# nmerty/nerf-fl

Hardware: AMD Instinct MI355X
Metric: ray-samples/sec (64+64) (higher is better)
Workload: dtype f16x3 fwd + f16 bwd; 1 GPU; configs[1]: lego-like rays, base NeRF coarse+fine, white_back; 4096 rays/GPU, N_samples=64 + N_importance=64, perturb=1 noise_std=1; train step: render_rays fwd + NerfWLoss + HIP backward + grad all-reduce + Adam + re-pack; rays_per_gpu=4096, mode=train, precision=f16x3, forward_arithmetic=fp16 MFMA, operands split hi+lo, 3 products, fp32 accumulate (f16x3), mlp_evals_per_ray=192, hip_graph=False, full=False

## Files before the change

### nerf_fl_amd/csrc/nfl_math.h

```cpp
#pragma once
#include <hip/hip_runtime.h>

#include "../../include/nerf_fl_amd.h"
#include "nfl_macros.h"

typedef float f4v __attribute__((ext_vector_type(4)));

template <class Cam>
NFL_DEV void nfl_cam_ray(const Cam& c, long long p, f4v& r0, f4v& r1) {
    const float i = (float)(p % c.width), j = (float)(p / c.width);
    const float dx = (i - c.cx) / c.fx, dy = -(j - c.cy) / c.fy, dz = -1.f;
    float d[3];
#pragma unroll
    for (int r = 0; r < 3; ++r) d[r] = dx * c.c2w[4 * r] + dy * c.c2w[4 * r + 1] + dz * c.c2w[4 * r + 2];
    const float n = sqrtf(d[0] * d[0] + d[1] * d[1] + d[2] * d[2]);
    r0 = f4v{c.c2w[3], c.c2w[7], c.c2w[11], d[0] / n};
    r1 = f4v{d[1] / n, d[2] / n, c.near, c.far};
}

NFL_DEV float nfl_softplus(float x) { return x > 20.f ? x : log1pf(expf(x)); }
NFL_DEV float nfl_sigmoid(float x) { return 1.f / (1.f + expf(-x)); }

NFL_DEV float nfl_sin_rev(float r) {
    r = r - rintf(r);
    float a = fabsf(r);
    a = a > 0.25f ? 0.5f - a : a;
    a = copysignf(a, r);
    const float a2 = a * a;
    float p = 3.953670604e+01f;
    p = __builtin_fmaf(p, a2, -7.654978229e+01f);
    p = __builtin_fmaf(p, a2, 8.160100407e+01f);
    p = __builtin_fmaf(p, a2, -4.134165503e+01f);
    p = __builtin_fmaf(p, a2, 6.283185160e+00f);
    return a * p;
}

NFL_DEV void nfl_turns(float x, float& th, float& tl) {
    const float C_HI = 0.15915493667125702f;
    const float C_LO = 6.4206382432985265e-09f;
    th = x * C_HI;
    const float e = __builtin_fmaf(x, C_HI, -th);
    tl = __builtin_fmaf(x, C_LO, e);
}

template <int N>
NFL_DEV float nfl_pe_feature(int f, const float (&raw)[3], const float (&th)[3], const float (&tl)[3], const float* pw) {
    if (f < 3) return raw[f];
    if (f >= 6 * N + 3) return 0.f;
    const int g = f - 3, k = g / 6, rem = g % 6, t = rem / 3, c = rem % 3;
    const float sc = (float)(1 << k);
    float r = __builtin_amdgcn_fractf(th[c] * sc) + tl[c] * sc;
    if (t) r += 0.25f;
    return pw[k] * nfl_sin_rev(r);
}

NFL_DEV float nfl_relu(float x) {
    int b = __builtin_bit_cast(int, x);
    b = b > 0 ? b : 0;
    return __builtin_bit_cast(float, b);
}
template <class E>
NFL_DEV unsigned nfl_pack2(float a, float b) {
    typedef E e2v __attribute__((ext_vector_type(2)));
    e2v r;
    r[0] = (E)a;
    r[1] = (E)b;
    return __builtin_bit_cast(unsigned, r);
}
template <class E>
NFL_DEV unsigned nfl_split_pair(float x0, float x1, float& l0, float& l1) {
    const unsigned hi = nfl_pack2<E>(x0, x1);
    if constexpr (__is_same(E, _Float16)) {
        asm("v_fma_mix_f32 %0, %1, -1.0, %2 op_sel_hi:[1,0,0]" : "=v"(l0) : "v"(hi), "v"(x0));
        asm("v_fma_mix_f32 %0, %1, -1.0, %2 op_sel:[1,0,0] op_sel_hi:[1,0,0]" : "=v"(l1) : "v"(hi), "v"(x1));
    } else {
        l0 = x0 - __builtin_bit_cast(float, hi << 16);
        asm volatile("" : "+v"(l0));
        l1 = x1 - __builtin_bit_cast(float, hi & 0xffff0000u);
    }
    return hi;
}

template <int NP>
NFL_DEV void nfl_split8(const float (&v)[8], h8 (&dst)[NP]) {
    using E = _Float16;
#pragma unroll
    for (int j = 0; j < 8; j += 2) {
        if constexpr (NP == 2) {
            float l0, l1;
            reinterpret_cast<unsigned(&)[4]>(dst[0])[j / 2] = nfl_split_pair<E>(v[j], v[j + 1], l0, l1);
            reinterpret_cast<unsigned(&)[4]>(dst[NP - 1])[j / 2] = nfl_pack2<E>(l0, l1);
        } else {
            reinterpret_cast<unsigned(&)[4]>(dst[0])[j / 2] = nfl_pack2<E>(v[j], v[j + 1]);
        }
    }
}
```

### nerf_fl_amd/csrc/nfl_mlp.h

```cpp
#pragma once
#include "nfl_dev.h"
#include "nfl_diag.h"
#include "nfl_math.h"
#include "nfl_plan.h"
#include "nfl_prods.h"

__device__ __forceinline__ f16v nfl_mfma(h8 a, h8 b, f16v c) { return __builtin_amdgcn_mfma_f32_32x32x16_f16(a, b, c, 0, 0, 0); }

#define NFL_STREAM_STORE(v, p) __builtin_nontemporal_store(v, p)

template <int LO = 0>
NFL_DEV void nfl_stash8(const float (&v)[8], char* dst) {
    h8 t, tl;
#pragma unroll
    for (int j = 0; j < 8; j += 2) {
        if constexpr (LO != 0) {
            float l0, l1;
            reinterpret_cast<unsigned(&)[4]>(t)[j / 2] = nfl_split_pair<_Float16>(v[j], v[j + 1], l0, l1);
            reinterpret_cast<unsigned(&)[4]>(tl)[j / 2] = nfl_pack2<_Float16>(l0, l1);
        } else {
            reinterpret_cast<unsigned(&)[4]>(t)[j / 2] = nfl_pack2<_Float16>(v[j], v[j + 1]);
        }
    }
    NFL_STREAM_STORE(t, reinterpret_cast<h8*>(dst));
    if constexpr (LO != 0) NFL_STREAM_STORE(tl, reinterpret_cast<h8*>(dst + LO));
}

template <int N, int NP, int LO = 0>
NFL_DEV void nfl_pe_kstep(int ks, int h, const float (&raw)[3], const float (&th)[3], const float (&tl)[3],
                          const float* pw, h8 (&dst)[NP], char* stash = nullptr) {
    float v[8];
#pragma unroll
    for (int j = 0; j < 8; ++j) {
        const int f0 = 16 * ks + j, f1 = f0 + 8;
        if (f0 < 3 || f0 >= 6 * N + 3 || f1 >= 6 * N + 3) {
            const float v0 = nfl_pe_feature<N>(f0, raw, th, tl, pw);
            const float v1 = nfl_pe_feature<N>(f1, raw, th, tl, pw);
            v[j] = h ? v1 : v0;
        } else {
            const int g0 = f0 - 3, g1 = f1 - 3;
            const int k0 = g0 / 6, k1 = g1 / 6, t0 = (g0 % 6) / 3, t1 = (g1 % 6) / 3, c0 = g0 % 3, c1 = g1 % 3;
            const float sc = h ? (float)(1 << k1) : (float)(1 << k0);
            const float thc = h ? th[c1] : th[c0];
            const float tlc = h ? tl[c1] : tl[c0];
            const float ph = h ? 0.25f * t1 : 0.25f * t0;
            const float r = __builtin_amdgcn_fractf(thc * sc) + tlc * sc + ph;
            v[j] = (h ? pw[k1] : pw[k0]) * nfl_sin_rev(r);
        }
    }
    nfl_split8<NP>(v, dst);
    if (stash) {
        NFL_STREAM_STORE(dst[0], reinterpret_cast<h8*>(stash));
        if constexpr (LO != 0 && NP == 2) NFL_STREAM_STORE(dst[NP - 1], reinterpret_cast<h8*>(stash + LO));
    }
}

template <int SLOT_BYTES, int MAXP_>
struct NflRing {
    static constexpr int MAXP = MAXP_;
    const char* gsrc;
    const int* chunk_off;
    char* lds;
    int n_chunks;
    int c_issue;
    int s_issue;
    int s_read;
    int wave, lane;
    const char* i_src;
    char* i_dst;
    int i_nbytes;

#ifdef NFL_STAMPS
    unsigned long long t_wait = 0, t_bar = 0;
#endif
    int n_off0, n_off1;
    unsigned ovf = 0;

    NFL_DEV void begin_issue() {
        i_nbytes = n_off1 - n_off0;
        i_src = gsrc + n_off0;
        i_dst = lds + s_issue * SLOT_BYTES;
        c_issue = c_issue + 1 == n_chunks ? 0 : c_issue + 1;
        s_issue = s_issue == 2 ? 0 : s_issue + 1;
        n_off0 = __builtin_amdgcn_readfirstlane(chunk_off[c_issue]);
        n_off1 = __builtin_amdgcn_readfirstlane(chunk_off[c_issue + 1]);
    }
    template <int P>
    NFL_DEV void piece() {
        if constexpr (P < MAXP) {
            unsigned byte = (unsigned)(wave + 4 * P) * 1024u;
            const unsigned last = (unsigned)i_nbytes - 1024u;
            byte = byte < last ? byte : last;
            const unsigned vo = byte + (threadIdx.x & 63) * 16u;
            __builtin_amdgcn_global_load_lds(
                (const __attribute__((address_space(1))) void*)(i_src + vo),
                (__attribute__((address_space(3))) void*)(i_dst + byte), 16, 0, 0);
        }
    }
    template <int P0, int P1>
    NFL_DEV void pieces() {
        nfl_static_for<P0, P1>([&](auto P) __attribute__((always_inline)) { piece<decltype(P)::value>(); });
    }
    NFL_DEV void prime() {
        n_off0 = __builtin_amdgcn_readfirstlane(chunk_off[c_issue]);
        n_off1 = __builtin_amdgcn_readfirstlane(chunk_off[c_issue + 1]);
        begin_issue();
        pieces<0, MAXP>();
        begin_issue();
        pieces<0, MAXP>();
    }
    template <int EXTRA = 0>
    NFL_DEV const char* consume() {
#if defined(NFL_STAMPS) && NFL_STAMPS >= 2
        const unsigned long long c0 = __builtin_amdgcn_s_memtime();
        asm volatile("s_waitcnt vmcnt(%0) lgkmcnt(0)" ::"n"(MAXP + EXTRA) : "memory");
        const unsigned long long c1 = __builtin_amdgcn_s_memtime();
        __builtin_amdgcn_s_barrier();
        t_wait += c1 - c0;
        t_bar += __builtin_amdgcn_s_memtime() - c1;
#else
        asm volatile("s_waitcnt vmcnt(%0) lgkmcnt(0)" ::"n"(MAXP + EXTRA) : "memory");
        __builtin_amdgcn_s_barrier();
#endif
        asm volatile("" ::: "memory");
        begin_issue();
        const char* base = lds + s_read * SLOT_BYTES + (threadIdx.x & 63) * 16;
        s_read = s_read == 2 ? 0 : s_read + 1;
        return base;
    }
};

template <int NP, int NCB>
NFL_DEV void nfl_bias_init(f16v (&acc)[NCB], const float* bias_rt, int h) {
#pragma unroll
    for (int q = 0; q < 4; ++q) {
        const f4v b = *reinterpret_cast<const f4v*>(bias_rt + 8 * q + 4 * h);
#pragma unroll
        for (int cb = 0; cb < NCB; ++cb) {
            acc[cb][4 * q + 0] = b[0];
            acc[cb][4 * q + 1] = b[1];
            acc[cb][4 * q + 2] = b[2];
            acc[cb][4 * q + 3] = b[3];
        }
    }
}

typedef unsigned nfl_u4 __attribute__((ext_vector_type(4)));
template <int OFF>
NFL_DEV nfl_u4 nfl_lds_read128(unsigned addr) {
    static_assert(OFF >= 0 && OFF < 65536, "ds_read offset field is 16 bits");
    nfl_u4 r;
    asm volatile("ds_read_b128 %0, %1 offset:%2" : "=v"(r) : "v"(addr), "n"(OFF));
    return r;
}
template <int N, int NREAD, int NWP>
NFL_DEV void nfl_lds_wait(nfl_u4 (&w)[NWP]) {
    if constexpr (NREAD == 2) asm volatile("s_waitcnt lgkmcnt(%2)" : "+v"(w[0]), "+v"(w[1]) : "n"(N));
    else asm volatile("s_waitcnt lgkmcnt(%1)" : "+v"(w[0]) : "n"(N));
}

#ifndef NFL_DEPTH_X3
#define NFL_DEPTH_X3 2
#endif
template <int PRODS, int NP, int NCB, int NK, int P0, class V8, class GetB, class Epi, class Ring,
          int DEPTH = ((NP == 1 && (PRODS & 4) == 0) ? 4 : NFL_DEPTH_X3)>
NFL_DEV void nfl_tile_p(f16v (&acc)[NCB], const char* wl, const int frag0, GetB&& getb, Epi&& epi, Ring& ring) {
    constexpr int NWP = (NP == 2 || (PRODS & 4) != 0) ? 2 : 1;
    constexpr int KSB = 1024 * NWP;
    constexpr int NW = DEPTH + 1;
    constexpr bool W_LO = NWP == 2 && (PRODS & 1) != 0, X_LO = NP == 2 && (PRODS & 2) != 0;
    constexpr int NREAD = W_LO ? 2 : 1;
    (void)frag0;
    nfl_u4 w[NW][NWP];
    const unsigned wa = (unsigned)(size_t)(__attribute__((address_space(3))) const char*)wl;
    auto load = [&](auto K) __attribute__((always_inline)) {
        constexpr int k = decltype(K)::value;
        w[k % NW][0] = nfl_lds_read128<(P0 + k) * KSB>(wa);
        if constexpr (W_LO) w[k % NW][NWP - 1] = nfl_lds_read128<(P0 + k) * KSB + 1024>(wa);
    };
    nfl_static_for<0, (DEPTH < NK ? DEPTH : NK)>([&](auto K) __attribute__((always_inline)) { load(K); });
    epi.early();
    __builtin_amdgcn_sched_barrier(0);
    nfl_static_for<0, NK>([&](auto K) __attribute__((always_inline)) {
        constexpr int k = decltype(K)::value;
        constexpr int younger = (NK - 1 - k) < (DEPTH - 1) ? (NK - 1 - k) : (DEPTH - 1);
        nfl_lds_wait<younger * NREAD, NREAD>(w[k % NW]);
#pragma unroll
        for (int cb = 0; cb < NCB; ++cb) {
            if constexpr (W_LO) {
                acc[cb] = nfl_mfma(__builtin_bit_cast(V8, w[k % NW][NWP - 1]), getb(K, cb, 0), acc[cb]);
                if (cb == 0) {
                    if constexpr (k + DEPTH < NK) load(std::integral_constant<int, k + DEPTH>{});
                }
                __builtin_amdgcn_sched_barrier(0);
            }
            if constexpr (X_LO) {
                acc[cb] = nfl_mfma(__builtin_bit_cast(V8, w[k % NW][0]), getb(K, cb, NP - 1), acc[cb]);
                if (cb == 0) {
                    if constexpr (!W_LO && k + DEPTH < NK) load(std::integral_constant<int, k + DEPTH>{});
                    ring.template piece<P0 + k>();
                }
                __builtin_amdgcn_sched_barrier(0);
            }
            acc[cb] = nfl_mfma(__builtin_bit_cast(V8, w[k % NW][0]), getb(K, cb, 0), acc[cb]);
            if (cb == 0) {
                if constexpr (!W_LO && !X_LO && k + DEPTH < NK) load(std::integral_constant<int, k + DEPTH>{});
                if constexpr (!X_LO) ring.template piece<P0 + k>();
            }
            if (cb == NCB - 1) epi.template step<k, NK>();
            __builtin_amdgcn_sched_barrier(0);
        }
    });
}
template <int NP, int NCB, int NK, int P0, class V8, class GetB, class Epi, class Ring>
NFL_DEV void nfl_tile(f16v (&acc)[NCB], const char* wl, const int frag0, GetB&& getb, Epi&& epi, Ring& ring) {
    nfl_tile_p<3, NP, NCB, NK, P0, V8>(acc, wl, frag0, getb, epi, ring);
}

struct NflNoEpi {
    template <int K, int NK> NFL_DEV void step() {}
    NFL_DEV void early() {}
};
#ifndef NFL_EPI_EARLY
#define NFL_EPI_EARLY 2
#endif

template <int NP, int NCB, bool RELU, bool STASH, int NOUT, int MSLOT, int LO = 0, bool ZST = false>
struct NflActEpi {
    const f16v (&acc)[NCB];
    h8 (&out)[NOUT][NCB][NP];
    const int ks;
    char* const (&stash)[NCB];
    const int slot;
    char* const (&mstash)[NCB];
    const int mword;
    unsigned (&mq)[NCB][4];
    unsigned& ovf;
    float* const* zc;
    const int zpad;
    h8 tmp[NCB];
    h8 tmpl[LO != 0 ? NCB : 1];
    unsigned m32[NCB];

    template <int OP>
    NFL_DEV void pair() {
        constexpr int s = OP / 4, j = 2 * (OP % 4);
#pragma unroll
        for (int cb = 0; cb < NCB; ++cb) {
            float x0 = acc[cb][8 * s + j], x1 = acc[cb][8 * s + j + 1];
            if constexpr (ZST) {
                const int f = 16 * (ks + s) + 8 * (j >> 2) + 4 * (int)((threadIdx.x & 63) >> 5) + (j & 3);
                zc[cb][(size_t)f * zpad] = x0;
                zc[cb][(size_t)(f + 1) * zpad] = x1;
            }
            if (RELU) {
                x0 = nfl_relu(x0);
                x1 = nfl_relu(x1);
            }
            unsigned hi;
            if constexpr (NP == 2) {
                float l0, l1;
                hi = nfl_split_pair<_Float16>(x0, x1, l0, l1);
                const unsigned lo = nfl_pack2<_Float16>(l0, l1);
                reinterpret_cast<unsigned(&)[4]>(out[ks + s][cb][NP - 1])[j / 2] = lo;
                if constexpr (STASH && LO != 0) {
                    reinterpret_cast<unsigned(&)[4]>(tmpl[cb])[j / 2] = lo;
                    if (OP % 4 == 3) NFL_STREAM_STORE(tmpl[cb], reinterpret_cast<h8*>(stash[cb] + LO + (slot + s) * 1024));
                }
            } else {
                hi = nfl_pack2<_Float16>(x0, x1);
            }
            reinterpret_cast<unsigned(&)[4]>(out[ks + s][cb][0])[j / 2] = hi;
            {
                const unsigned mag = RELU ? hi : (hi & 0x7fff7fffu);
                asm("v_pk_max_u16 %0, %0, %1" : "+v"(ovf) : "v"(mag));
            }
            if (STASH) {
                reinterpret_cast<unsigned(&)[4]>(tmp[cb])[j / 2] = hi;
                if (OP % 4 == 3) NFL_STREAM_STORE(tmp[cb], reinterpret_cast<h8*>(stash[cb] + (slot + s) * 1024));
                if (RELU) {
                    unsigned on;
                    asm("v_pk_min_u16 %0, %1, %2" : "=v"(on) : "v"(hi), "s"(0x00010001u));
                    m32[cb] = OP == 0 ? on : ((on << (2 * OP)) | m32[cb]);
                    if (OP == 7) {
                        mq[cb][MSLOT] = m32[cb];
                        if (MSLOT == 3) {
                            typedef unsigned nfl_mq4 __attribute__((ext_vector_type(4)));
                            const nfl_mq4 v = {mq[cb][0], mq[cb][1], mq[cb][2], mq[cb][3]};
                            NFL_STREAM_STORE(v, reinterpret_cast<nfl_mq4*>(mstash[cb] + (mword >> 2) * 1024));
                        }
                    }
                }
            }
        }
    }
    template <int K, int NK>
    NFL_DEV void step() {
        constexpr int R = 8 - NFL_EPI_EARLY;
        nfl_static_for<NFL_EPI_EARLY + (R * K) / NK, NFL_EPI_EARLY + (R * (K + 1)) / NK>([&](auto O) __attribute__((always_inline)) {
            pair<decltype(O)::value>();
        });
    }
    NFL_DEV void early() {
        nfl_static_for<0, NFL_EPI_EARLY>([&](auto O) __attribute__((always_inline)) { pair<decltype(O)::value>(); });
    }
    NFL_DEV void all() {
        nfl_static_for<0, 8>([&](auto O) __attribute__((always_inline)) { pair<decltype(O)::value>(); });
    }
};

template <int NP, int NCB, int NKA, int NKB, bool RELU, int NRT, int TPC, bool STASH, int LO = 0, int PRODS = 3, bool ZST = false, int NINA, int NINB, int NOUT, class Ring>
NFL_DEV void nfl_dense(Ring& ring, const float* bias_lds, int& rt, int h,
                       const h8 (&inA)[NINA][NCB][NP], int ksA0,
                       const h8 (&inB)[NINB][NCB][NP], int ksB0,
                       h8 (&out)[NOUT][NCB][NP], int out_ks0, char* const (&stash)[NCB], int slot0,
                       char* const (&mstash)[NCB], int mw0, float* const* zc = nullptr, int zpad = 0) {
    constexpr int NK = NKA + NKB;
    constexpr int NST = 2 * NCB * (LO != 0 ? 2 : 1);
    unsigned mq[NCB][4];
    f16v acc[2][NCB];
    const char* wl = nullptr;
    auto getb = [&](auto K, int cb, int part) __attribute__((always_inline)) -> const h8& {
        constexpr int k = decltype(K)::value;
        if constexpr (k < NKA) return inA[ksA0 + k][cb][part];
        else return inB[ksB0 + k - NKA][cb][part];
    };
    nfl_static_for<0, NRT>([&](auto I) __attribute__((always_inline)) {
        constexpr int i = decltype(I)::value;
        if (i % TPC == 0) wl = ring.template consume<(STASH && TPC == 1 && i >= 2) ? NST : 0>();
        constexpr int frag0 = (i % TPC) * NK;
        nfl_bias_init<NP, NCB>(acc[i & 1], bias_lds + (rt + i) * 32, h);
        if constexpr (i > 0) {
            NflActEpi<NP, NCB, RELU, STASH, NOUT, (i - 1) & 3, LO, ZST> epi{acc[(i - 1) & 1], out, out_ks0 + 2 * (i - 1), stash, slot0 + 2 * (i - 1), mstash, mw0 + i - 1, mq, ring.ovf, zc, zpad};
            nfl_tile_p<PRODS, NP, NCB, NK, frag0, h8>(acc[i & 1], wl, frag0, getb, epi, ring);
        } else {
            NflNoEpi epi;
            nfl_tile_p<PRODS, NP, NCB, NK, frag0, h8>(acc[i & 1], wl, frag0, getb, epi, ring);
        }
        if (i % TPC == TPC - 1 || i == NRT - 1) ring.template pieces<((i % TPC) + 1) * NK, Ring::MAXP>();
    });
    NflActEpi<NP, NCB, RELU, STASH, NOUT, (NRT - 1) & 3, LO, ZST> last{acc[(NRT - 1) & 1], out, out_ks0 + 2 * (NRT - 1), stash, slot0 + 2 * (NRT - 1), mstash, mw0 + NRT - 1, mq, ring.ovf, zc, zpad};
    last.all();
    rt += NRT;
}

template <int NP, int NCB, int NK, int PRODS = 3, int NIN, class Ring>
NFL_DEV void nfl_head(Ring& ring, const float* bias_lds, int& rt, int h,
                      const h8 (&in)[NIN][NCB][NP], int ks0, f16v (&acc)[NCB]) {
    const char* wl = ring.consume();
    nfl_bias_init<NP, NCB>(acc, bias_lds + rt * 32, h);
    auto getb = [&](auto K, int cb, int part) __attribute__((always_inline)) -> const h8& {
        return in[ks0 + decltype(K)::value][cb][part];
    };
    NflNoEpi epi;
    nfl_tile_p<PRODS, NP, NCB, NK, 0, h8>(acc, wl, 0, getb, epi, ring);
    ring.template pieces<NK, Ring::MAXP>();
    rt += 1;
}
```

### nerf_fl_amd/csrc/nfl_render_impl.h

```cpp
#pragma once
#include "nfl_launch.h"
#include "nfl_mlp.h"

#define NFL_NST 20
#define NFL_REC 32

template <class PA>
NFL_DEV float nfl_z_plain(const PA& a, float near, float far, int i) {
    const float s = a.d_lin[i];
    const float oms = 1.0f - s;
    if (!a.use_disp) return near * oms + far * s;
    return 1.0f / (1.0f / near * oms + 1.0f / far * s);
}
template <class PA>
NFL_DEV float nfl_z_at(const PA& a, int ray, float near, float far, int i) {
    const int N = a.n_samples;
    if (a.d_z) return a.d_z[(size_t)ray * N + i];
    float z = nfl_z_plain(a, near, far, i);
    if (a.perturb > 0.f) {
        const float zm = nfl_z_plain(a, near, far, i > 0 ? i - 1 : 0);
        const float zp = nfl_z_plain(a, near, far, i < N - 1 ? i + 1 : N - 1);
        const float upper = i < N - 1 ? 0.5f * (z + zp) : z;
        const float lower = i > 0 ? 0.5f * (zm + z) : z;
        const float pr = a.perturb * a.d_perturb_rand[(size_t)ray * N + i];
        z = lower + (upper - lower) * pr;
    }
    return z;
}

template <int NSPLIT, int NCB, int NFX>
struct NflRenderCfg {
    static constexpr int NP = NSPLIT == 3 ? 2 : 1;
    static constexpr int NKP = (6 * NFX + 3 + 15) / 16;
    static constexpr int KSB = 1024 * NP;
    static constexpr int MAXKS = 16 + (NKP > 5 ? NKP : 5);
    static constexpr int SLOT = MAXKS * KSB;
    static constexpr int MAXP = (SLOT + 4095) / 4096;
    static constexpr int NSLOT = 4 * NCB;
    static constexpr int LDS_RING = 3 * SLOT;
    static constexpr int LDS_BIAS = NFL_MAX_RT * 32 * 4;
    static constexpr int LDS_REC = (NSLOT + 2) * NFL_REC * 4;
    static constexpr int LDS_CHK = (NFL_MAX_CHUNKS + 8 + 32 + 8) * 4;
    static constexpr int LDS_BYTES = LDS_RING + LDS_BIAS + LDS_REC + LDS_CHK;
};

#ifdef NFL_STAMPS
#include "nfl_stamps.h"
#define NFL_STAMP(i)                                                      \
    do {                                                                  \
        const unsigned long long t_now = __builtin_amdgcn_s_memtime();    \
        t_acc[i] += t_now - t_last;                                       \
        t_last = t_now;                                                   \
    } while (0)
#else
#define NFL_STAMP(i) do {} while (0)
#endif

#define NFL_LOSS_ON(a) ((a).d_loss_target != nullptr)
typedef NflKernarg<RenderArgs> NflKArgs;
NFL_DEV NflKArgs nfl_kargs() { return nfl_kernarg<RenderArgs>(); }

typedef const __attribute__((address_space(4))) nfl_camera* NflKCam;
NFL_DEV NflKCam nfl_kcam(NflKArgs K) {
    return K->a.d_cam ? (NflKCam)(unsigned long long)K->a.d_cam : &K->cam;
}

template <int NSPLIT, int NCB, int NFX, int MODE>
__global__ __launch_bounds__(256, 1) void nfl_render_kernel(const RenderArgs A) {
    constexpr bool STASH = MODE == NFL_MODE_STASH || MODE == NFL_MODE_STASH2, EMBED = MODE == NFL_MODE_EMBED;
    constexpr bool ZC = MODE == NFL_MODE_ZCACHE;
    using C = NflRenderCfg<NSPLIT, NCB, NFX>;
    constexpr int NP = C::NP, NKP = C::NKP, NSLOT = C::NSLOT;
    constexpr int SMULT = MODE == NFL_MODE_STASH2 ? 2 : 1;
    constexpr int LO = MODE == NFL_MODE_STASH2 ? nfl_act_slots(NKP) * 1024 : 0;
    extern __shared__ __attribute__((aligned(16))) char smem[];
    float* const bias_lds = reinterpret_cast<float*>(smem);
    float* const rec_lds = reinterpret_cast<float*>(smem + C::LDS_BIAS);
    int* const chk_lds = reinterpret_cast<int*>(smem + C::LDS_BIAS + C::LDS_REC);
    float* const pw_lds = reinterpret_cast<float*>(chk_lds + NFL_MAX_CHUNKS + 8);
    float* const loss_lds = pw_lds + 32;

    const nfl_pass_args& a = A.a;
    const int tid = threadIdx.x;
    const int lane = tid & 63;
    const int wave = __builtin_amdgcn_readfirstlane(tid >> 6);
    const int h = lane >> 5, c = lane & 31;
    const int N = a.n_samples, SPR = A.spr;

    const int ray0 = blockIdx.x * A.rays_per_wg;
    int ray1 = ray0 + A.rays_per_wg;
    if (ray1 > a.n_rays) ray1 = a.n_rays;
    if (ray0 >= ray1) return;
    const int seg_end = (ray1 - ray0) * SPR;
    const int ntiles = (seg_end + NSLOT - 1) / NSLOT;

    {
        const float* bg = reinterpret_cast<const float*>(A.packed + A.bias_off);
        for (int i = tid; i < A.n_rt * 32; i += 256) bias_lds[i] = bg[i];
        for (int i = tid; i <= A.n_chunks; i += 256) chk_lds[i] = A.plan->chunk_off[i];
        if (tid < 16) pw_lds[tid] = (a.d_pe_w_xyz && tid < A.nfx_rt) ? a.d_pe_w_xyz[tid] : 1.f;
        else if (tid < 32) pw_lds[tid] = (a.d_pe_w_dir && tid - 16 < A.ndir_rt) ? a.d_pe_w_dir[tid - 16] : 1.f;
        else if (tid < 36) loss_lds[tid - 32] = 0.f;
    }
    __syncthreads();

    NflRing<C::SLOT, C::MAXP> ring;
    ring.gsrc = A.packed;
    ring.chunk_off = chk_lds;
    ring.lds = smem + C::LDS_BIAS + C::LDS_REC + C::LDS_CHK;
    ring.n_chunks = A.n_chunks;
    ring.c_issue = 0;
    ring.s_issue = 0;
    ring.s_read = 0;
    ring.wave = wave;
    ring.lane = lane;
    ring.prime();

#ifdef NFL_STAMPS
    unsigned long long t_acc[NFL_NSTAMP] = {};
    unsigned long long t_last = __builtin_amdgcn_s_memtime();
#endif
    for (int tile = 0; tile < ntiles; ++tile) {
        NflKArgs K = nfl_kargs();
        int s_ray[NCB], s_idx[NCB];
        bool s_ok[NCB];
        float s_z[NCB], s_dl[NCB];
        h8 P[NKP][NCB][NP];
        h8 X[16][NCB][NP], Y[16][NCB][NP];
        char* st[NCB];
        char* mst[NCB];
        float* zc[NCB];
#pragma unroll
        for (int cb = 0; cb < NCB; ++cb) {
            const int g = tile * NSLOT + wave * NCB + cb;
            const bool seg_ok = g < seg_end;
            const int gg = seg_ok ? g : seg_end - 1;
            const int ray = ray0 + gg / SPR;
            const int i = (gg % SPR) * 32 + c;
            const bool ok = seg_ok && i < N;
            const int ii = i < N ? i : N - 1;
            if constexpr (EMBED) {
                const int b = ray * 32 + c;
                const bool pok = seg_ok && b < K->n_points;
                const float* xr = K->a.d_embedded + (size_t)(b < K->n_points ? b : K->n_points - 1) * K->emb_stride;
                st[cb] = nullptr;
                mst[cb] = nullptr;
                s_ray[cb] = ray;
                s_idx[cb] = c;
                s_ok[cb] = pok;
                s_z[cb] = 0.f;
                s_dl[cb] = 0.f;
#pragma unroll
                for (int ks = 0; ks < NKP; ++ks) {
                    float v[8];
#pragma unroll
                    for (int j = 0; j < 8; ++j) {
                        const int f = 16 * ks + 8 * h + j;
                        v[j] = f < K->cx ? xr[f] : 0.f;
                    }
                    nfl_split8<NP>(v, P[ks][cb]);
                }
                continue;
            }
            f4v r0, r1;
            if (K->gen_rays) {
                const NflKCam cam = nfl_kcam(K);
                nfl_cam_ray(*cam, cam->pix0 + ray, r0, r1);
            } else
            {
                const float* rp = K->a.d_rays + (size_t)ray * 8;
                r0 = *reinterpret_cast<const f4v*>(rp);
                r1 = *reinterpret_cast<const f4v*>(rp + 4);
            }
            const float near = r1[2], far = r1[3];
            const float z = nfl_z_at(K->a, ray, near, far, ii);
            const float zn = ii + 1 < N ? nfl_z_at(K->a, ray, near, far, ii + 1) : z;
            st[cb] = STASH ? K->a.d_act_stash + ((size_t)(ray0 * SPR + gg) * nfl_act_rec(NKP, SMULT)) * 1024 + (2 * c + h) * 16
                           : nullptr;
            mst[cb] = STASH ? K->a.d_act_stash + nfl_msk_offset((size_t)K->a.n_rays * SPR, NKP, SMULT)
                                  + (size_t)(ray0 * SPR + gg) * (NFL_MSK_WORDS * 256) + lane * 16
                            : nullptr;
            s_ray[cb] = ray;
            s_idx[cb] = ii;
            s_ok[cb] = ok;
            zc[cb] = ZC ? K->zcache + (size_t)ray * 128 * K->zpad + ii : nullptr;
            s_z[cb] = z;
            s_dl[cb] = ii + 1 < N ? zn - z : 1e2f;
            if (K->a.d_z_out && ok && h == 0) K->a.d_z_out[(size_t)ray * N + ii] = z;
            float raw[3], th[3], tl[3];
            raw[0] = r0[0] + r0[3] * z;
            raw[1] = r0[1] + r1[0] * z;
            raw[2] = r0[2] + r1[1] * z;
#pragma unroll
            for (int k = 0; k < 3; ++k) nfl_turns(raw[k], th[k], tl[k]);
#pragma unroll
            for (int ks = 0; ks < NKP; ++ks) {
                nfl_pe_kstep<NFX, NP, LO>(ks, h, raw, th, tl, pw_lds, P[ks][cb], STASH ? st[cb] + ks * 1024 : nullptr);
                __builtin_amdgcn_sched_barrier(0);
            }
        }

        K = nfl_kargs();
        int rt = 0;
        float o_sig[NCB], o_rgb[NCB][3], o_tr[NCB][5];
        NFL_STAMP(0);
        nfl_dense<NP, NCB, NKP, 0, true, 8, 2, STASH, LO, NFL_PRODS[NFL_P_IDX_L1]>(ring, bias_lds, rt, h, P, 0, P, 0, X, 0, st, nfl_act_h(NKP, 1), mst, nfl_msk_h(1));
        NFL_STAMP(1);
        nfl_dense<NP, NCB, 16, 0, true, 8, 1, STASH, LO, NFL_PRODS[NFL_P_IDX_L2]>(ring, bias_lds, rt, h, X, 0, X, 0, Y, 0, st, nfl_act_h(NKP, 2), mst, nfl_msk_h(2));
        NFL_STAMP(2);
        nfl_dense<NP, NCB, 16, 0, true, 8, 1, STASH, LO, NFL_PRODS[NFL_P_IDX_L3]>(ring, bias_lds, rt, h, Y, 0, Y, 0, X, 0, st, nfl_act_h(NKP, 3), mst, nfl_msk_h(3));
        NFL_STAMP(3);
        nfl_dense<NP, NCB, 16, 0, true, 8, 1, STASH, LO, NFL_PRODS[NFL_P_IDX_L4]>(ring, bias_lds, rt, h, X, 0, X, 0, Y, 0, st, nfl_act_h(NKP, 4), mst, nfl_msk_h(4));
        NFL_STAMP(4);
        nfl_dense<NP, NCB, NKP, 16, true, 8, 1, STASH, LO, NFL_PRODS[NFL_P_IDX_L5]>(ring, bias_lds, rt, h, P, 0, Y, 0, X, 0, st, nfl_act_h(NKP, 5), mst, nfl_msk_h(5));
        NFL_STAMP(5);
        nfl_dense<NP, NCB, 16, 0, true, 8, 1, STASH, LO, NFL_PRODS[NFL_P_IDX_L6]>(ring, bias_lds, rt, h, X, 0, X, 0, Y, 0, st, nfl_act_h(NKP, 6), mst, nfl_msk_h(6));
        NFL_STAMP(6);
        nfl_dense<NP, NCB, 16, 0, true, 8, 1, STASH, LO, NFL_PRODS[NFL_P_IDX_L7]>(ring, bias_lds, rt, h, Y, 0, Y, 0, X, 0, st, nfl_act_h(NKP, 7), mst, nfl_msk_h(7));
        NFL_STAMP(7);
        nfl_dense<NP, NCB, 16, 0, true, 8, 1, STASH, LO, NFL_PRODS[NFL_P_IDX_L8]>(ring, bias_lds, rt, h, X, 0, X, 0, Y, 0, st, nfl_act_h(NKP, 8), mst, nfl_msk_h(8));
        NFL_STAMP(8);
        {
            f16v hacc[NCB];
            nfl_head<NP, NCB, 16, NFL_PRODS[NFL_P_IDX_SIG]>(ring, bias_lds, rt, h, Y, 0, hacc);
#pragma unroll
            for (int cb = 0; cb < NCB; ++cb) o_sig[cb] = hacc[cb][0];
        }
        NFL_STAMP(9);
        K = nfl_kargs();
        if (!K->a.sigma_only) {
            NFL_STAMP(10);
            {
                h8 D[5][NCB][NP];
#pragma unroll
                for (int cb = 0; cb < NCB; ++cb) {
                    if constexpr (EMBED) {
                        const int b = s_ray[cb] * 32 + s_idx[cb];
                        const float* xr = K->a.d_embedded + (size_t)(b < K->n_points ? b : K->n_points - 1) * K->emb_stride
                                          + K->cx;
#pragma unroll
                        for (int ks = 0; ks < 5; ++ks) {
                            if (ks >= 2 && !K->has_a) break;
                            float v[8];
#pragma unroll
                            for (int j = 0; j < 8; ++j) {
                                const int f = 16 * (ks < 2 ? ks : ks - 2) + 8 * h + j;
                                v[j] = ks < 2 ? (f < K->cd ? xr[f] : 0.f) : (f < K->n_a ? xr[K->cd + f] : 0.f);
                            }
                            nfl_split8<NP>(v, D[ks][cb]);
                        }
                        continue;
                    }
                    float raw[3], th[3], tl[3];
                    if (K->gen_rays && !K->a.d_view_dir) {
                        f4v g0, g1;
                        const NflKCam cam = nfl_kcam(K);
                        nfl_cam_ray(*cam, cam->pix0 + s_ray[cb], g0, g1);
                        raw[0] = g0[3];
                        raw[1] = g1[0];
                        raw[2] = g1[1];
                    } else {
                        const float* dp = K->a.d_view_dir ? K->a.d_view_dir + (size_t)s_ray[cb] * 3
                                                       : K->a.d_rays + (size_t)s_ray[cb] * 8 + 3;
#pragma unroll
                        for (int k = 0; k < 3; ++k) raw[k] = dp[k];
                    }
#pragma unroll
                    for (int k = 0; k < 3; ++k) nfl_turns(raw[k], th[k], tl[k]);
                    char* sd = STASH ? st[cb] + nfl_act_d(NKP) * 1024 : nullptr;
                    nfl_pe_kstep<4, NP, LO>(0, h, raw, th, tl, pw_lds + 16, D[0][cb], sd);
                    __builtin_amdgcn_sched_barrier(0);
                    nfl_pe_kstep<4, NP, LO>(1, h, raw, th, tl, pw_lds + 16, D[1][cb], STASH ? sd + 1024 : nullptr);
                    __builtin_amdgcn_sched_barrier(0);
                    if (K->has_a) {
                        const int na = K->n_a;
                        const float* ap = K->a.d_a_emb + (size_t)s_ray[cb] * na + 8 * h;
#pragma unroll
                        for (int ks = 0; ks < 3; ++ks) {
                            float v[8];
                            if (na == 48) {
                                const f4v v0 = *reinterpret_cast<const f4v*>(ap + 16 * ks);
                                const f4v v1 = *reinterpret_cast<const f4v*>(ap + 16 * ks + 4);
                                v[0] = v0[0]; v[1] = v0[1]; v[2] = v0[2]; v[3] = v0[3];
                                v[4] = v1[0]; v[5] = v1[1]; v[6] = v1[2]; v[7] = v1[3];
                            } else {
#pragma unroll
                                for (int j = 0; j < 8; ++j) v[j] = 16 * ks + 8 * h + j < na ? ap[16 * ks + j] : 0.f;
                            }
                            nfl_split8<NP>(v, D[2 + ks][cb]);
                            if (STASH) nfl_stash8<LO>(v, sd + (2 + ks) * 1024);
                        }
                    }
                }
                NFL_STAMP(11);
                if (K->has_a)
                    nfl_dense<NP, NCB, 16, 5, true, 4, 1, STASH, LO, NFL_PRODS[NFL_P_IDX_DIR], ZC>(ring, bias_lds, rt, h, Y, 0, D, 0, X, 0, st, nfl_act_dirh(NKP), mst, nfl_msk_dirh(), zc, ZC ? K->zpad : 0);
                else
                    nfl_dense<NP, NCB, 16, 2, true, 4, 1, STASH, LO, NFL_PRODS[NFL_P_IDX_DIR], ZC>(ring, bias_lds, rt, h, Y, 0, D, 0, X, 0, st, nfl_act_dirh(NKP), mst, nfl_msk_dirh(), zc, ZC ? K->zpad : 0);
            }
            NFL_STAMP(12);
            {
                f16v hacc[NCB];
                nfl_head<NP, NCB, 8, NFL_PRODS[NFL_P_IDX_RGB]>(ring, bias_lds, rt, h, X, 0, hacc);
// ... 287 lines not shown
```

Measured before the change: 112.8 million ray-samples/s.

## Interleave next tile's ray setup and positional encoding into trunk layers 6-8

Moves per-tile ray generation, z sampling and positional-encoding computation for the next tile into small slices. The slices are hooked into the k-step loop of dense layers 6-8 of the current tile, so VALU setup work overlaps with MFMA and ring loads instead of running serially at the start of each tile. The first tile is prepared before the loop, and P now persists across iterations. This adds register pressure (extra per-cb state kept live across layers) and a complex static hook schedule, which could cause spills or disturb the tuned MFMA pipeline.

After: 112.9 million ray-samples/s (median of 2 runs). About the same (+0.1%).

```diff
diff --git a/nerf_fl_amd/csrc/nfl_math.h b/nerf_fl_amd/csrc/nfl_math.h
--- a/nerf_fl_amd/csrc/nfl_math.h
+++ b/nerf_fl_amd/csrc/nfl_math.h
@@ -21,11 +21,13 @@
 NFL_DEV float nfl_softplus(float x) { return x > 20.f ? x : log1pf(expf(x)); }
 NFL_DEV float nfl_sigmoid(float x) { return 1.f / (1.f + expf(-x)); }
 
-NFL_DEV float nfl_sin_rev(float r) {
+NFL_DEV float nfl_sin_fold(float r) {
     r = r - rintf(r);
     float a = fabsf(r);
     a = a > 0.25f ? 0.5f - a : a;
-    a = copysignf(a, r);
+    return copysignf(a, r);
+}
+NFL_DEV float nfl_sin_poly(float a) {
     const float a2 = a * a;
     float p = 3.953670604e+01f;
     p = __builtin_fmaf(p, a2, -7.654978229e+01f);
@@ -34,6 +36,7 @@
     p = __builtin_fmaf(p, a2, 6.283185160e+00f);
     return a * p;
 }
+NFL_DEV float nfl_sin_rev(float r) { return nfl_sin_poly(nfl_sin_fold(r)); }
 
 NFL_DEV void nfl_turns(float x, float& th, float& tl) {
     const float C_HI = 0.15915493667125702f;
@@ -44,14 +47,18 @@
 }
 
 template <int N>
-NFL_DEV float nfl_pe_feature(int f, const float (&raw)[3], const float (&th)[3], const float (&tl)[3], const float* pw) {
+NFL_DEV float nfl_pe_feature_w(int f, const float (&raw)[3], const float (&th)[3], const float (&tl)[3], float pwk) {
     if (f < 3) return raw[f];
     if (f >= 6 * N + 3) return 0.f;
     const int g = f - 3, k = g / 6, rem = g % 6, t = rem / 3, c = rem % 3;
     const float sc = (float)(1 << k);
     float r = __builtin_amdgcn_fractf(th[c] * sc) + tl[c] * sc;
     if (t) r += 0.25f;
-    return pw[k] * nfl_sin_rev(r);
+    return pwk * nfl_sin_rev(r);
+}
+template <int N>
+NFL_DEV float nfl_pe_feature(int f, const float (&raw)[3], const float (&th)[3], const float (&tl)[3], const float* pw) {
+    return nfl_pe_feature_w<N>(f, raw, th, tl, (f < 3 || f >= 6 * N + 3) ? 0.f : pw[(f - 3) / 6]);
 }
 
 NFL_DEV float nfl_relu(float x) {
diff --git a/nerf_fl_amd/csrc/nfl_mlp.h b/nerf_fl_amd/csrc/nfl_mlp.h
--- a/nerf_fl_amd/csrc/nfl_mlp.h
+++ b/nerf_fl_amd/csrc/nfl_mlp.h
@@ -26,28 +26,52 @@
     if constexpr (LO != 0) NFL_STREAM_STORE(tl, reinterpret_cast<h8*>(dst + LO));
 }
 
+template <int N>
+NFL_DEV constexpr bool nfl_pe_both_sines(int ks, int j) {
+    const int f0 = 16 * ks + j, f1 = f0 + 8;
+    return !(f0 < 3 || f0 >= 6 * N + 3 || f1 >= 6 * N + 3);
+}
+NFL_DEV float nfl_pick3(int c, float a0, float a1, float a2) { return c == 0 ? a0 : (c == 1 ? a1 : a2); }
+template <int N>
+NFL_DEV float nfl_pe_arg(int ks, int j, int h, float th0, float th1, float th2, float tl0, float tl1, float tl2) {
+    const int f0 = 16 * ks + j, f1 = f0 + 8;
+    if (!nfl_pe_both_sines<N>(ks, j)) return 0.f;
+    const int g0 = f0 - 3, g1 = f1 - 3;
+    const int k0 = g0 / 6, k1 = g1 / 6, t0 = (g0 % 6) / 3, t1 = (g1 % 6) / 3, c0 = g0 % 3, c1 = g1 % 3;
+    const float sc = h ? (float)(1 << k1) : (float)(1 << k0);
+    const float thc = h ? nfl_pick3(c1, th0, th1, th2) : nfl_pick3(c0, th0, th1, th2);
+    const float tlc = h ? nfl_pick3(c1, tl0, tl1, tl2) : nfl_pick3(c0, tl0, tl1, tl2);
+    const float ph = h ? 0.25f * t1 : 0.25f * t0;
+    return __builtin_amdgcn_fractf(thc * sc) + tlc * sc + ph;
+}
+template <int N>
+NFL_DEV float nfl_pe_arg(int ks, int j, int h, const float (&th)[3], const float (&tl)[3]) {
+    return nfl_pe_arg<N>(ks, j, h, th[0], th[1], th[2], tl[0], tl[1], tl[2]);
+}
+template <int N>
+NFL_DEV constexpr int nfl_pe_freq(int ks, int j, int half) {
+    const int f = 16 * ks + j + 8 * half;
+    return (f < 3 || f >= 6 * N + 3) ? 0 : (f - 3) / 6;
+}
+template <int N>
+NFL_DEV float nfl_pe_val(int ks, int j, int h, float a, const float (&raw)[3], const float (&th)[3], const float (&tl)[3],
+                         float pw0, float pw1) {
+    const int f0 = 16 * ks + j, f1 = f0 + 8;
+    if (!nfl_pe_both_sines<N>(ks, j)) {
+        const float v0 = nfl_pe_feature_w<N>(f0, raw, th, tl, pw0);
+        const float v1 = nfl_pe_feature_w<N>(f1, raw, th, tl, pw1);
+        return h ? v1 : v0;
+    }
+    return (h ? pw1 : pw0) * nfl_sin_poly(a);
+}
 template <int N, int NP, int LO = 0>
 NFL_DEV void nfl_pe_kstep(int ks, int h, const float (&raw)[3], const float (&th)[3], const float (&tl)[3],
                           const float* pw, h8 (&dst)[NP], char* stash = nullptr) {
     float v[8];
 #pragma unroll
-    for (int j = 0; j < 8; ++j) {
-        const int f0 = 16 * ks + j, f1 = f0 + 8;
-        if (f0 < 3 || f0 >= 6 * N + 3 || f1 >= 6 * N + 3) {
-            const float v0 = nfl_pe_feature<N>(f0, raw, th, tl, pw);
-            const float v1 = nfl_pe_feature<N>(f1, raw, th, tl, pw);
-            v[j] = h ? v1 : v0;
-        } else {
-            const int g0 = f0 - 3, g1 = f1 - 3;
-            const int k0 = g0 / 6, k1 = g1 / 6, t0 = (g0 % 6) / 3, t1 = (g1 % 6) / 3, c0 = g0 % 3, c1 = g1 % 3;
-            const float sc = h ? (float)(1 << k1) : (float)(1 << k0);
-            const float thc = h ? th[c1] : th[c0];
-            const float tlc = h ? tl[c1] : tl[c0];
-            const float ph = h ? 0.25f * t1 : 0.25f * t0;
-            const float r = __builtin_amdgcn_fractf(thc * sc) + tlc * sc + ph;
-            v[j] = (h ? pw[k1] : pw[k0]) * nfl_sin_rev(r);
-        }
-    }
+    for (int j = 0; j < 8; ++j)
+        v[j] = nfl_pe_val<N>(ks, j, h, nfl_sin_fold(nfl_pe_arg<N>(ks, j, h, th, tl)), raw, th, tl,
+                             pw[nfl_pe_freq<N>(ks, j, 0)], pw[nfl_pe_freq<N>(ks, j, 1)]);
     nfl_split8<NP>(v, dst);
     if (stash) {
         NFL_STREAM_STORE(dst[0], reinterpret_cast<h8*>(stash));
@@ -162,6 +186,7 @@
 #ifndef NFL_DEPTH_X3
 #define NFL_DEPTH_X3 2
 #endif
+struct NflHasMid {};
 template <int PRODS, int NP, int NCB, int NK, int P0, class V8, class GetB, class Epi, class Ring,
           int DEPTH = ((NP == 1 && (PRODS & 4) == 0) ? 4 : NFL_DEPTH_X3)>
 NFL_DEV void nfl_tile_p(f16v (&acc)[NCB], const char* wl, const int frag0, GetB&& getb, Epi&& epi, Ring& ring) {
@@ -199,6 +224,7 @@
                 if (cb == 0) {
                     if constexpr (!W_LO && k + DEPTH < NK) load(std::integral_constant<int, k + DEPTH>{});
                     ring.template piece<P0 + k>();
+                    if constexpr (std::is_base_of<NflHasMid, std::remove_reference_t<Epi>>::value) epi.template mid<k, NK>();
                 }
                 __builtin_amdgcn_sched_barrier(0);
             }
@@ -224,6 +250,25 @@
 #ifndef NFL_EPI_EARLY
 #define NFL_EPI_EARLY 2
 #endif
+struct NflNoSide {
+    template <int I, int K, int NK> NFL_DEV void mid() {}
+    template <int I, int K, int NK> NFL_DEV void step() {}
+};
+template <int I, bool MID, class Epi, class Side>
+struct NflEpiSide : NflHasMid {
+    Epi& epi;
+    Side& side;
+    NFL_DEV NflEpiSide(Epi& e, Side& s) : epi(e), side(s) {}
+    template <int K, int NK> NFL_DEV void mid() {
+        if constexpr (MID) side.template mid<I, K, NK>();
+    }
+    template <int K, int NK> NFL_DEV void step() {
+        epi.template step<K, NK>();
+        if constexpr (!MID) side.template mid<I, K, NK>();
+        side.template step<I, K, NK>();
+    }
+    NFL_DEV void early() { epi.early(); }
+};
 
 template <int NP, int NCB, bool RELU, bool STASH, int NOUT, int MSLOT, int LO = 0, bool ZST = false>
 struct NflActEpi {
@@ -309,12 +354,14 @@
     }
 };
 
-template <int NP, int NCB, int NKA, int NKB, bool RELU, int NRT, int TPC, bool STASH, int LO = 0, int PRODS = 3, bool ZST = false, int NINA, int NINB, int NOUT, class Ring>
-NFL_DEV void nfl_dense(Ring& ring, const float* bias_lds, int& rt, int h,
-                       const h8 (&inA)[NINA][NCB][NP], int ksA0,
-                       const h8 (&inB)[NINB][NCB][NP], int ksB0,
-                       h8 (&out)[NOUT][NCB][NP], int out_ks0, char* const (&stash)[NCB], int slot0,
-                       char* const (&mstash)[NCB], int mw0, float* const* zc = nullptr, int zpad = 0) {
+template <int NP, int NCB, int NKA, int NKB, bool RELU, int NRT, int TPC, bool STASH, int LO = 0, int PRODS = 3, bool ZST = false, int NINA, int NINB, int NOUT, class Ring, class Side>
+NFL_DEV void nfl_dense_side(Ring& ring, const float* bias_lds, int& rt, int h,
+                            const h8 (&inA)[NINA][NCB][NP], int ksA0,
+                            const h8 (&inB)[NINB][NCB][NP], int ksB0,
+                            h8 (&out)[NOUT][NCB][NP], int out_ks0, char* const (&stash)[NCB], int slot0,
+                            char* const (&mstash)[NCB], int mw0, float* const* zc, int zpad, Side& side) {
+    constexpr bool SIDE = !std::is_same<Side, NflNoSide>::value;
+    constexpr bool MID = NP == 2 && (PRODS & 2) != 0;
     constexpr int NK = NKA + NKB;
     constexpr int NST = 2 * NCB * (LO != 0 ? 2 : 1);
     unsigned mq[NCB][4];
@@ -332,16 +379,36 @@
         nfl_bias_init<NP, NCB>(acc[i & 1], bias_lds + (rt + i) * 32, h);
         if constexpr (i > 0) {
             NflActEpi<NP, NCB, RELU, STASH, NOUT, (i - 1) & 3, LO, ZST> epi{acc[(i - 1) & 1], out, out_ks0 + 2 * (i - 1), stash, slot0 + 2 * (i - 1), mstash, mw0 + i - 1, mq, ring.ovf, zc, zpad};
-            nfl_tile_p<PRODS, NP, NCB, NK, frag0, h8>(acc[i & 1], wl, frag0, getb, epi, ring);
+            if constexpr (SIDE) {
+                NflEpiSide<i, MID, decltype(epi), Side> es(epi, side);
+                nfl_tile_p<PRODS, NP, NCB, NK, frag0, h8>(acc[i & 1], wl, frag0, getb, es, ring);
+            } else {
+                nfl_tile_p<PRODS, NP, NCB, NK, frag0, h8>(acc[i & 1], wl, frag0, getb, epi, ring);
+            }
         } else {
             NflNoEpi epi;
-            nfl_tile_p<PRODS, NP, NCB, NK, frag0, h8>(acc[i & 1], wl, frag0, getb, epi, ring);
+            if constexpr (SIDE) {
+                NflEpiSide<i, MID, NflNoEpi, Side> es(epi, side);
+                nfl_tile_p<PRODS, NP, NCB, NK, frag0, h8>(acc[i & 1], wl, frag0, getb, es, ring);
+            } else {
+                nfl_tile_p<PRODS, NP, NCB, NK, frag0, h8>(acc[i & 1], wl, frag0, getb, epi, ring);
+            }
         }
         if (i % TPC == TPC - 1 || i == NRT - 1) ring.template pieces<((i % TPC) + 1) * NK, Ring::MAXP>();
     });
     NflActEpi<NP, NCB, RELU, STASH, NOUT, (NRT - 1) & 3, LO, ZST> last{acc[(NRT - 1) & 1], out, out_ks0 + 2 * (NRT - 1), stash, slot0 + 2 * (NRT - 1), mstash, mw0 + NRT - 1, mq, ring.ovf, zc, zpad};
     last.all();
     rt += NRT;
+}
+template <int NP, int NCB, int NKA, int NKB, bool RELU, int NRT, int TPC, bool STASH, int LO = 0, int PRODS = 3, bool ZST = false, int NINA, int NINB, int NOUT, class Ring>
+NFL_DEV void nfl_dense(Ring& ring, const float* bias_lds, int& rt, int h,
+                       const h8 (&inA)[NINA][NCB][NP], int ksA0,
+                       const h8 (&inB)[NINB][NCB][NP], int ksB0,
+                       h8 (&out)[NOUT][NCB][NP], int out_ks0, char* const (&stash)[NCB], int slot0,
+                       char* const (&mstash)[NCB], int mw0, float* const* zc = nullptr, int zpad = 0) {
+    NflNoSide side;
+    nfl_dense_side<NP, NCB, NKA, NKB, RELU, NRT, TPC, STASH, LO, PRODS, ZST>(ring, bias_lds, rt, h, inA, ksA0, inB, ksB0, out, out_ks0,
+                                                                           stash, slot0, mstash, mw0, zc, zpad, side);
 }
 
 template <int NP, int NCB, int NK, int PRODS = 3, int NIN, class Ring>
diff --git a/nerf_fl_amd/csrc/nfl_render_impl.h b/nerf_fl_amd/csrc/nfl_render_impl.h
--- a/nerf_fl_amd/csrc/nfl_render_impl.h
+++ b/nerf_fl_amd/csrc/nfl_render_impl.h
@@ -65,6 +65,160 @@
     return K->a.d_cam ? (NflKCam)(unsigned long long)K->a.d_cam : &K->cam;
 }
 
+#define NFL_SIDE_K0 11
+#define NFL_SIDE_GAP 16
+template <int NSPLIT, int NCB, int NFX, int MODE>
+struct NflTileSetup {
+    static constexpr bool STASH = MODE == NFL_MODE_STASH || MODE == NFL_MODE_STASH2, ZC = MODE == NFL_MODE_ZCACHE;
+    using C = NflRenderCfg<NSPLIT, NCB, NFX>;
+    static constexpr int NP = C::NP, NKP = C::NKP, NSLOT = C::NSLOT;
+    static constexpr int SMULT = MODE == NFL_MODE_STASH2 ? 2 : 1;
+    static constexpr int LO = MODE == NFL_MODE_STASH2 ? nfl_act_slots(NKP) * 1024 : 0;
+    static constexpr int NS = 2 + 28 * NKP;
+    static constexpr int HPT = 8, NH = 3 * 8 * HPT;
+    static constexpr int hook_of(int k, bool mid) {
+        constexpr int K0 = NFL_SIDE_K0;
+        return k == K0 ? (mid ? 0 : 1) : k == K0 + 1 ? (mid ? 2 : 3) : k == K0 + 2 ? (mid ? 4 : -1) : k == K0 + 3 ? (mid ? 5 : 6)
+             : k == K0 + 4 ? (mid ? 7 : -1) : -1;
+    }
+
+    int tile;
+    const int ray0, seg_end, SPR, N, wave, lane;
+    const float* const pw_lds;
+    int (&s_ray)[NCB], (&s_idx)[NCB];
+    bool (&s_ok)[NCB];
+    float (&s_z)[NCB], (&s_dl)[NCB];
+    char* (&st)[NCB];
+    char* (&mst)[NCB];
+    float* (&zc)[NCB];
+    h8 (&P)[NKP][NCB][NP];
+    f4v r0[NCB], r1[NCB];
+    float zn[NCB];
+    float raw[NCB][3], th[NCB][3], tl[NCB][3];
+    float arg[NCB], v0[NCB], v1[NCB];
+    float pws[NFX];
+
+    template <int S>
+    NFL_DEV void slice() {
+        const int h = lane >> 5, c = lane & 31;
+        if constexpr (S == 0) {
+            NflKArgs K = nfl_kargs();
+#pragma unroll
+            for (int cb = 0; cb < NCB; ++cb) {
+                const int g = tile * NSLOT + wave * NCB + cb;
+                const bool seg_ok = g < seg_end;
+                const int gg = seg_ok ? g : seg_end - 1;
+                const int ray = ray0 + gg / SPR;
+                const int i = (gg % SPR) * 32 + c;
+                const bool ok = seg_ok && i < N;
+                const int ii = i < N ? i : N - 1;
+                if (K->gen_rays) {
+                    const NflKCam cam = nfl_kcam(K);
+                    nfl_cam_ray(*cam, cam->pix0 + ray, r0[cb], r1[cb]);
+                } else {
+                    const float* rp = K->a.d_rays + (size_t)ray * 8;
+                    r0[cb] = *reinterpret_cast<const f4v*>(rp);
+                    r1[cb] = *reinterpret_cast<const f4v*>(rp + 4);
+                }
+                if (K->a.d_z) {
+                    s_z[cb] = K->a.d_z[(size_t)ray * N + ii];
+                    zn[cb] = ii + 1 < N ? K->a.d_z[(size_t)ray * N + ii + 1] : 0.f;
+                }
+                st[cb] = STASH ? K->a.d_act_stash + ((size_t)(ray0 * SPR + gg) * nfl_act_rec(NKP, SMULT)) * 1024 + (2 * c + h) * 16
+                               : nullptr;
+                mst[cb] = STASH ? K->a.d_act_stash + nfl_msk_offset((size_t)K->a.n_rays * SPR, NKP, SMULT)
+                                      + (size_t)(ray0 * SPR + gg) * (NFL_MSK_WORDS * 256) + lane * 16
+                                : nullptr;
+                s_ray[cb] = ray;
+                s_idx[cb] = ii;
+                s_ok[cb] = ok;
+                zc[cb] = ZC ? K->zcache + (size_t)ray * 128 * K->zpad + ii : nullptr;
+            }
+        } else if constexpr (S == 1) {
+            NflKArgs K = nfl_kargs();
+#pragma unroll
+            for (int cb = 0; cb < NCB; ++cb) {
+                const int ray = s_ray[cb], ii = s_idx[cb];
+                const float near = r1[cb][2], far = r1[cb][3];
+                float z = s_z[cb], zq = zn[cb];
+                if (!K->a.d_z) {
+                    z = nfl_z_at(K->a, ray, near, far, ii);
+                    zq = ii + 1 < N ? nfl_z_at(K->a, ray, near, far, ii + 1) : z;
+                }
+                s_z[cb] = z;
+                s_dl[cb] = ii + 1 < N ? zq - z : 1e2f;
+                if (K->a.d_z_out && s_ok[cb] && h == 0) K->a.d_z_out[(size_t)ray * N + ii] = z;
+                raw[cb][0] = r0[cb][0] + r0[cb][3] * z;
+                raw[cb][1] = r0[cb][1] + r1[cb][0] * z;
+                raw[cb][2] = r0[cb][2] + r1[cb][1] * z;
+#pragma unroll
+                for (int k = 0; k < 3; ++k) nfl_turns(raw[cb][k], th[cb][k], tl[cb][k]);
+            }
+#pragma unroll
+            for (int k = 0; k < NFX; ++k)
+                pws[k] = __builtin_bit_cast(float, __builtin_amdgcn_readfirstlane(__builtin_bit_cast(int, pw_lds[k])));
+        } else {
+            constexpr int ks = (S - 2) / 28, p = ((S - 2) % 28) / 7, q = (S - 2) % 7, j = 2 * p + (q >= 3);
+#pragma unroll
+            for (int cb = 0; cb < NCB; ++cb) {
+                if constexpr (q == 0 || q == 3) {
+                    arg[cb] = nfl_pe_arg<NFX>(ks, j, h, th[cb][0], th[cb][1], th[cb][2], tl[cb][0], tl[cb][1], tl[cb][2]);
+                    asm volatile("" : "+v"(arg[cb]));
+                } else if constexpr (q == 1 || q == 4) {
+                    arg[cb] = nfl_sin_fold(arg[cb]);
+                    asm volatile("" : "+v"(arg[cb]));
+                } else if constexpr (q == 2 || q == 5) {
+                    const float lraw[3] = {raw[cb][0], raw[cb][1], raw[cb][2]};
+                    const float lth[3] = {th[cb][0], th[cb][1], th[cb][2]};
+                    const float ltl[3] = {tl[cb][0], tl[cb][1], tl[cb][2]};
+                    const float v = nfl_pe_val<NFX>(ks, j, h, arg[cb], lraw, lth, ltl, pws[nfl_pe_freq<NFX>(ks, j, 0)],
+                                                    pws[nfl_pe_freq<NFX>(ks, j, 1)]);
+                    if constexpr (q == 2) v0[cb] = v;
+                    else v1[cb] = v;
+                    asm volatile("" : "+v"(q == 2 ? v0[cb] : v1[cb]));
+                } else {
+                    if constexpr (NP == 2) {
+                        float l0, l1;
+                        reinterpret_cast<unsigned(&)[4]>(P[ks][cb][0])[p] = nfl_split_pair<_Float16>(v0[cb], v1[cb], l0, l1);
+                        reinterpret_cast<unsigned(&)[4]>(P[ks][cb][NP - 1])[p] = nfl_pack2<_Float16>(l0, l1);
+                    } else {
+                        reinterpret_cast<unsigned(&)[4]>(P[ks][cb][0])[p] = nfl_pack2<_Float16>(v0[cb], v1[cb]);
+                    }
+                    if constexpr (STASH && p == 3) {
+                        NFL_STREAM_STORE(P[ks][cb][0], reinterpret_cast<h8*>(st[cb] + ks * 1024));
+                        if constexpr (LO != 0 && NP == 2) NFL_STREAM_STORE(P[ks][cb][NP - 1], reinterpret_cast<h8*>(st[cb] + ks * 1024 + LO));
+                    }
+                }
+            }
+        }
+    }
+    NFL_DEV void all() {
+        nfl_static_for<0, NS>([&](auto S) __attribute__((always_inline)) {
+            slice<decltype(S)::value>();
+            if constexpr (decltype(S)::value >= 2 && (decltype(S)::value - 2) % 28 == 27) __builtin_amdgcn_sched_barrier(0);
+        });
+    }
+    static constexpr int first_slice(int g) {
+        return g <= 0 ? 0 : g <= NFL_SIDE_GAP ? 1 : 1 + ((g - NFL_SIDE_GAP) * (NS - 1)) / (NH - NFL_SIDE_GAP);
+    }
+    template <int G>
+    NFL_DEV void hook() {
+        nfl_static_for<first_slice(G), first_slice(G + 1)>([&](auto S) __attribute__((always_inline)) { slice<decltype(S)::value>(); });
+    }
+};
+template <int L, class Setup>
+struct NflSetupSide {
+    Setup& su;
+    template <int I, int K, int NK> NFL_DEV void mid() { at<I, Setup::hook_of(K, true)>(); }
+    template <int I, int K, int NK> NFL_DEV void step() {
+        static_assert(NK == 16, "hooks are laid out for the 16 k-steps of a trunk layer");
+        at<I, Setup::hook_of(K, false)>();
+    }
+    template <int I, int H> NFL_DEV void at() {
+        if constexpr (H >= 0) su.template hook<(L * 8 + I) * Setup::HPT + H>();
+    }
+};
+
 template <int NSPLIT, int NCB, int NFX, int MODE>
 __global__ __launch_bounds__(256, 1) void nfl_render_kernel(const RenderArgs A) {
     constexpr bool STASH = MODE == NFL_MODE_STASH || MODE == NFL_MODE_STASH2, EMBED = MODE == NFL_MODE_EMBED;
@@ -120,25 +274,43 @@
     unsigned long long t_acc[NFL_NSTAMP] = {};
     unsigned long long t_last = __builtin_amdgcn_s_memtime();
 #endif
+    constexpr bool PIPE = !EMBED;
+    h8 P[NKP][NCB][NP];
+    int n_ray[NCB], n_idx[NCB];
+    bool n_ok[NCB];
+    float n_z[NCB], n_dl[NCB];
+    char* n_st[NCB];
+    char* n_mst[NCB];
+    float* n_zc[NCB];
+    NflTileSetup<NSPLIT, NCB, NFX, MODE> su{0, ray0, seg_end, SPR, N, wave, lane, pw_lds,
+                                            n_ray, n_idx, n_ok, n_z, n_dl, n_st, n_mst, n_zc, P};
+    if constexpr (PIPE) su.all();
     for (int tile = 0; tile < ntiles; ++tile) {
         NflKArgs K = nfl_kargs();
         int s_ray[NCB], s_idx[NCB];
         bool s_ok[NCB];
         float s_z[NCB], s_dl[NCB];
-        h8 P[NKP][NCB][NP];
         h8 X[16][NCB][NP], Y[16][NCB][NP];
         char* st[NCB];
         char* mst[NCB];
         float* zc[NCB];
 #pragma unroll
         for (int cb = 0; cb < NCB; ++cb) {
+            if constexpr (PIPE) {
+                s_ray[cb] = n_ray[cb];
+                s_idx[cb] = n_idx[cb];
+                s_ok[cb] = n_ok[cb];
+                s_z[cb] = n_z[cb];
+                s_dl[cb] = n_dl[cb];
+                st[cb] = n_st[cb];
+                mst[cb] = n_mst[cb];
+                zc[cb] = n_zc[cb];
+                continue;
+            }
             const int g = tile * NSLOT + wave * NCB + cb;
             const bool seg_ok = g < seg_end;
             const int gg = seg_ok ? g : seg_end - 1;
             const int ray = ray0 + gg / SPR;
-            const int i = (gg % SPR) * 32 + c;
-            const bool ok = seg_ok && i < N;
-            const int ii = i < N ? i : N - 1;
             if constexpr (EMBED) {
                 const int b = ray * 32 + c;
                 const bool pok = seg_ok && b < K->n_points;
@@ -160,43 +332,6 @@
                     }
                     nfl_split8<NP>(v, P[ks][cb]);
                 }
-                continue;
-            }
-            f4v r0, r1;
-            if (K->gen_rays) {
-                const NflKCam cam = nfl_kcam(K);
-                nfl_cam_ray(*cam, cam->pix0 + ray, r0, r1);
-            } else
-            {
-                const float* rp = K->a.d_rays + (size_t)ray * 8;
-                r0 = *reinterpret_cast<const f4v*>(rp);
-                r1 = *reinterpret_cast<const f4v*>(rp + 4);
-            }
-            const float near = r1[2], far = r1[3];
-            const float z = nfl_z_at(K->a, ray, near, far, ii);
-            const float zn = ii + 1 < N ? nfl_z_at(K->a, ray, near, far, ii + 1) : z;
-            st[cb] = STASH ? K->a.d_act_stash + ((size_t)(ray0 * SPR + gg) * nfl_act_rec(NKP, SMULT)) * 1024 + (2 * c + h) * 16
-                           : nullptr;
-            mst[cb] = STASH ? K->a.d_act_stash + nfl_msk_offset((size_t)K->a.n_rays * SPR, NKP, SMULT)
-                                  + (size_t)(ray0 * SPR + gg) * (NFL_MSK_WORDS * 256) + lane * 16
-                            : nullptr;
-            s_ray[cb] = ray;
-            s_idx[cb] = ii;
-            s_ok[cb] = ok;
-            zc[cb] = ZC ? K->zcache + (size_t)ray * 128 * K->zpad + ii : nullptr;
-            s_z[cb] = z;
-            s_dl[cb] = ii + 1 < N ? zn - z : 1e2f;
-            if (K->a.d_z_out && ok && h == 0) K->a.d_z_out[(size_t)ray * N + ii] = z;
-            float raw[3], th[3], tl[3];
-            raw[0] = r0[0] + r0[3] * z;
-            raw[1] = r0[1] + r1[0] * z;
-            raw[2] = r0[2] + r1[1] * z;
-#pragma unroll
-            for (int k = 0; k < 3; ++k) nfl_turns(raw[k], th[k], tl[k]);
-#pragma unroll
-            for (int ks = 0; ks < NKP; ++ks) {
-                nfl_pe_kstep<NFX, NP, LO>(ks, h, raw, th, tl, pw_lds, P[ks][cb], STASH ? st[cb] + ks * 1024 : nullptr);
-                __builtin_amdgcn_sched_barrier(0);
             }
         }
 
@@ -214,11 +349,23 @@
         NFL_STAMP(4);
         nfl_dense<NP, NCB, NKP, 16, true, 8, 1, STASH, LO, NFL_PRODS[NFL_P_IDX_L5]>(ring, bias_lds, rt, h, P, 0, Y, 0, X, 0, st, nfl_act_h(NKP, 5), mst, nfl_msk_h(5));
         NFL_STAMP(5);
-        nfl_dense<NP, NCB, 16, 0, true, 8, 1, STASH, LO, NFL_PRODS[NFL_P_IDX_L6]>(ring, bias_lds, rt, h, X, 0, X, 0, Y, 0, st, nfl_act_h(NKP, 6), mst, nfl_msk_h(6));
-        NFL_STAMP(6);
-        nfl_dense<NP, NCB, 16, 0, true, 8, 1, STASH, LO, NFL_PRODS[NFL_P_IDX_L7]>(ring, bias_lds, rt, h, Y, 0, Y, 0, X, 0, st, nfl_act_h(NKP, 7), mst, nfl_msk_h(7));
-        NFL_STAMP(7);
-        nfl_dense<NP, NCB, 16, 0, true, 8, 1, STASH, LO, NFL_PRODS[NFL_P_IDX_L8]>(ring, bias_lds, rt, h, X, 0, X, 0, Y, 0, st, nfl_act_h(NKP, 8), mst, nfl_msk_h(8));
+        if constexpr (PIPE) {
+            su.tile = tile + 1;
+            NflSetupSide<0, decltype(su)> s6{su};
+            NflSetupSide<1, decltype(su)> s7{su};
+            NflSetupSide<2, decltype(su)> s8{su};
+            nfl_dense_side<NP, NCB, 16, 0, true, 8, 1, STASH, LO, NFL_PRODS[NFL_P_IDX_L6]>(ring, bias_lds, rt, h, X, 0, X, 0, Y, 0, st, nfl_act_h(NKP, 6), mst, nfl_msk_h(6), nullptr, 0, s6);
+            NFL_STAMP(6);
+            nfl_dense_side<NP, NCB, 16, 0, true, 8, 1, STASH, LO, NFL_PRODS[NFL_P_IDX_L7]>(ring, bias_lds, rt, h, Y, 0, Y, 0, X, 0, st, nfl_act_h(NKP, 7), mst, nfl_msk_h(7), nullptr, 0, s7);
+            NFL_STAMP(7);
+            nfl_dense_side<NP, NCB, 16, 0, true, 8, 1, STASH, LO, NFL_PRODS[NFL_P_IDX_L8]>(ring, bias_lds, rt, h, X, 0, X, 0, Y, 0, st, nfl_act_h(NKP, 8), mst, nfl_msk_h(8), nullptr, 0, s8);
+        } else {
+            nfl_dense<NP, NCB, 16, 0, true, 8, 1, STASH, LO, NFL_PRODS[NFL_P_IDX_L6]>(ring, bias_lds, rt, h, X, 0, X, 0, Y, 0, st, nfl_act_h(NKP, 6), mst, nfl_msk_h(6));
+            NFL_STAMP(6);
+            nfl_dense<NP, NCB, 16, 0, true, 8, 1, STASH, LO, NFL_PRODS[NFL_P_IDX_L7]>(ring, bias_lds, rt, h, Y, 0, Y, 0, X, 0, st, nfl_act_h(NKP, 7), mst, nfl_msk_h(7));
+            NFL_STAMP(7);
+            nfl_dense<NP, NCB, 16, 0, true, 8, 1, STASH, LO, NFL_PRODS[NFL_P_IDX_L8]>(ring, bias_lds, rt, h, X, 0, X, 0, Y, 0, st, nfl_act_h(NKP, 8), mst, nfl_msk_h(8));
+        }
         NFL_STAMP(8);
         {
             f16v hacc[NCB];
```
